# danielbrathwaite/OpenGL-Path-Tracing

Measured on AMD Instinct MI355X. Metric: Mrays/sec + ms/frame @1920×1080, 8 bounces, 1/2/4/8 MI355X, higher is better.
Workload: dtype f32; 1 GPU; C2: cornell 1920x1080, 1024 spp (frames 1..1024), 8 bounces (i<=8), AA+sky+sphere on; scene=cornell, width=1920, height=1080, spp=1024, max_bounce=8, frames_per_launch=1024, kernel_variant=0, parallelism=single GPU

## Files before the change

include/pt_api.h:

```cpp
#ifndef PT_API_H
#define PT_API_H

#include <stddef.h>

#ifdef __cplusplus
extern "C" {
#endif

#define PT_OK 0
#define PT_E_ARG (-1)
#define PT_E_IO (-2)
#define PT_E_PARSE (-3)
#define PT_E_SCENE (-4)
#define PT_E_HIP (-5)
#define PT_E_STATE (-6)

#define PT_FLAG_NO_AA 1
#define PT_FLAG_NO_SKY 2
#define PT_FLAG_NO_SPHERES 4
#define PT_FLAG_NO_TRIANGLES 8
#define PT_FLAG_REF_DISPATCH 16
#define PT_FLAG_MOLLER_TRUMBORE 32
#define PT_FLAG_ALL 63

// ... 26 lines not shown
int pt_progressive_setup(pt_ctx* ctx, int frames_per_launch, int launches_per_replay);
int pt_progressive_reset(pt_ctx* ctx, int next_frame);
int pt_progressive_run(pt_ctx* ctx, int replays);

int pt_rows(const pt_ctx* ctx, int* rows_local, int* row0, int* row_stride);
int pt_get_config(const pt_ctx* ctx, pt_config* out);

int pt_read_rgba32f(pt_ctx* ctx, float* host_dst, size_t bytes);
int pt_read_rgba8_aces(pt_ctx* ctx, unsigned char* host_dst, size_t bytes);
int pt_present_begin(pt_ctx* ctx, int buf);
int pt_present_end(pt_ctx* ctx, int buf, const unsigned char** pixels);
int pt_write_rgba32f(pt_ctx* ctx, const float* host_src, size_t bytes);

int pt_accum_device(pt_ctx* ctx, void** dev_ptr, size_t* bytes);
int pt_copy_rows_device(pt_ctx* ctx, void* dst_dev, size_t bytes);
int pt_stream(pt_ctx* ctx, void** stream);

int pt_set_counting(pt_ctx* ctx, int enable);
int pt_stats(pt_ctx* ctx, double* kernel_ms, unsigned long long out[5]);
int pt_stats_ex(pt_ctx* ctx, unsigned long long out[16]);
int pt_debug_launches(pt_ctx* ctx, unsigned long long out[2]);
int pt_debug_window_cull(pt_ctx* ctx, int* active, float* slack);
int pt_debug_sweep(pt_ctx* ctx, int* swept, int* qualifies, int* n_leaves);
int pt_debug_tile_order(pt_ctx* ctx, unsigned long long* sorts, unsigned* perm_out, int max_tiles, int* n_tiles,
                        int* tiles_x);
int pt_timing(pt_ctx* ctx, double* total_kernel_ms, int* n_launches, int reset);

int pt_set_kernel(pt_ctx* ctx, int variant);
int pt_set_tuning(pt_ctx* ctx, int key, int value);

typedef struct {
    unsigned long long pixels;
    unsigned long long sum_q;
    unsigned long long above;
    unsigned int max_q;
    int frames;
} pt_noise_stats;

int pt_set_moments(pt_ctx* ctx, int enable);
int pt_read_moments(pt_ctx* ctx, float* host_dst, size_t bytes, int* frames);
int pt_noise(pt_ctx* ctx, float target, pt_noise_stats* out);
int pt_noise_host(const float* moments, const unsigned char* in_footprint, size_t n_pixels, int frames,
                  float target, pt_noise_stats* out);
int pt_render_until(pt_ctx* ctx, int frame_first, int accumulate_first, int batch, int max_frames,
                    float target, int* frames_done, pt_noise_stats* last);

// ... 17 lines not shown
```

opengl-path-tracing_amd/csrc/pt_launch_plan.cpp:

```cpp
#include "pt_launch_plan.h"

#include "../../include/pt_api.h"

#include <algorithm>
#include <cmath>

namespace ptl {

static int resident_waves(int minw, bool lds) { return minw ? minw : (lds ? 7 : 6); }

static bool lds_staged(const SceneFacts& f, const Tuning& t, const Image& im, const State& s) {
    if (t.variant == 3) return false;
    if (f.lds_bytes <= kLdsSceneSmall) return true;
    return !s.counting && !t.minw && im.rpp == 1 && f.lds_bytes <= kLdsSceneMax;
}

bool cons_walk_on(const SceneFacts& f, const Tuning& t, bool counting) {
    if (!f.walk_nested || t.cons_off || counting) return false;
    const size_t mw = (size_t)resident_waves(t.minw, true);
    const auto blocks = [mw](size_t b) { return b ? std::min(mw, kLdsCu / b) : mw; };
    return blocks(f.lds_bytes_sk) >= blocks(f.lds_bytes);
}

bool window_cull_on(const SceneFacts& f, const Tuning& t, int flags, bool counting) {
// ... 120 lines not shown
    }
    if (p.overlap && p.nt == 256) {
        const int bpc = t.overlap_bpc ? t.overlap_bpc
                      : t.overlap_slots >= 3 ? (s.aces_fuse ? std::max(1, p.mw - 2) : 3)
                                             : std::max(1, p.mw - 1);
        p.blocks = std::min<unsigned>(p.blocks, (unsigned)(bpc * im.n_cu));
    }
    p.n_top = p.mw > 6 ? std::min(f.n_top, (int)kLdsCu / p.mw / 32 - 8) : f.n_top;
    const size_t shade_bytes = (size_t)(3 * f.n_mats + 2 * f.n_spheres) * 16;
    p.shade_lds = shade_bytes <= 4096;
    const size_t shade_lds_bytes = p.shade_lds ? shade_bytes : 0;
    if (p.wide) {
        const size_t blocks_cu = wide_nt == 1024 ? 1
                               : (wide_nt == 256 ? (size_t)(im.rpp > 1 ? 6 : std::min(std::max(p.mw, 5), 7))
                                                 : (size_t)(6 * 256 / wide_nt));
        p.wide_top = (int)std::min<size_t>({(size_t)f.n_wide, (size_t)kWideTopMax,
                                            (kLdsCu / blocks_cu - shade_lds_bytes - 1024) / 48});
    }
    p.dyn_lds_bytes = p.lds ? lds : (p.wide ? (size_t)p.wide_top * 48 : (size_t)p.n_top * 32) + shade_lds_bytes;
    p.key = kernel_key(s.counting, p.lds, p.wide, p.split, p.mw, im.rpp, p.nt, f.walk_np);
    p.common = !s.adaptive && common_launch(f, t, im, p);
    p.sweep = p.lds && p.nt == 256 && sweep_on(f, t, s.counting);
    if (p.sweep && !t.shade_thresh) p.shade_thresh = kSweepShadeThresh;
    if (p.split) {
        p.accum_long = n_frames > kShortLaunch;
        p.accum_moments = s.moments;
        p.aces_out = s.aces_fuse && !graph;
        const long long px = (long long)im.rows_local * im.width, per_block = 256 * (p.accum_long ? kAccumPixLong : kAccumPix);
        p.accum_blocks = (unsigned)((px + per_block - 1) / per_block);
    }
    return p;
}

size_t scratch_bytes(const LaunchPlan& plan, const Image& im, int n_frames) {
    if (!plan.split) return 0;
    return (size_t)std::max(im.rows_local, 1) * (size_t)im.width * (size_t)n_frames * 3 * sizeof(float);
}

}
```

opengl-path-tracing_amd/csrc/pt_launch_plan.h:

```cpp
#pragma once

#include <stddef.h>

namespace ptl {

#ifndef PT_PAD_NODES
#define PT_PAD_NODES 67
#endif
constexpr int kPadNodes = PT_PAD_NODES;
constexpr unsigned kPullBatch = 32;

constexpr size_t kLdsCu = 160 * 1024;
constexpr size_t kLdsSceneMax = 152 * 1024;
constexpr size_t kLdsSceneSmall = 48 * 1024;
constexpr int kShortLaunch = 16;
constexpr int kWideTopMax = 1 << 14;
constexpr int kWideThreadsAuto = 256;
constexpr int kMaxSlots = 4, kAutoSlots = 3;
#ifndef PT_ACCUM_PIX
#define PT_ACCUM_PIX 4
#endif
constexpr int kAccumPix = PT_ACCUM_PIX, kAccumPixLong = 2;
#ifndef PT_SWEEP_MAX_LEAVES
#define PT_SWEEP_MAX_LEAVES 24
#endif
constexpr int kSweepMaxLeaves = PT_SWEEP_MAX_LEAVES;
static_assert(kSweepMaxLeaves >= 1 && kSweepMaxLeaves <= 32, "a lane's candidate set is one 32-bit mask");
#ifndef PT_SWEEP_SHADE_THRESH
#define PT_SWEEP_SHADE_THRESH 56
#endif
constexpr int kSweepShadeThresh = PT_SWEEP_SHADE_THRESH;

struct SceneFacts {
    int n_nodes = 0, n_spheres = 0, n_mats = 0, n_slots = 0, n_top = 0, walk_np = 1, scene_fast = 0;
    bool walk_nested = false;
    bool wide_ok = false;
    int n_wide = 0;
    bool leaf_cert_ok = false;
    size_t lds_bytes = 0, lds_bytes_sk = 0;
    float root_box[6] = {0, 0, 0, 0, 0, 0};
    int root_child = -1;
    float cons_m[3] = {0, 0, 0};
    float win_slack[3] = {0, 0, 0};
    bool win_bad = false;
    float wide_cw[3] = {0, 0, 0};
    int n_leaves = 0;
    bool sweep_ok = false;
};

struct Tuning {
    int leaf_thresh = 0, shade_thresh = 0, minw = 0, trav_floor = 0, compact_max = 63, pull_batch = 0;
    int group_force = 0;
    int cons_off = 0;
    int wide_off = 0;
    int wide_threads = 0;
    int overlap_bpc = 0;
    int cert_off = 0;
    int overlap_slots = kAutoSlots;
    size_t scratch_budget = 0;
    int variant = 0;
    bool adaptive = true;
    int common_off = 0;
    int win_off = 0;
    int sweep_off = 0;
};

struct Image {
    int width, rows_local, n_tiles, rpp, flags, n_cu;
    unsigned persist_blocks;
    int tile_shift = 0;
};
struct State {
    bool counting, moments, aces_fuse;
    bool adaptive = false;
};

struct KernelKey { bool count, lds; int minw; bool multi, split, padn; int nt; bool wide; };
inline bool operator==(const KernelKey& a, const KernelKey& b) {
    return a.count == b.count && a.lds == b.lds && a.minw == b.minw && a.multi == b.multi && a.split == b.split &&
           a.padn == b.padn && a.nt == b.nt && a.wide == b.wide;
}

struct LaunchPlan {
    bool lds, wide, cons_walk, leaf_cert, split, overlap, shade_lds;
    int nt, mw, group, pull_batch, leaf_thresh, shade_thresh, trav_floor, n_top, wide_top;
    unsigned grp_magic, blocks;
    size_t dyn_lds_bytes;
    bool accum_long, accum_moments, aces_out;
    unsigned accum_blocks;
    KernelKey key;
    bool common;
    bool sweep;
};

constexpr KernelKey kCommonKey = {false, true, 7, false, true, true, 256, false};

bool cons_walk_on(const SceneFacts& f, const Tuning& t, bool counting);
bool window_cull_on(const SceneFacts& f, const Tuning& t, int flags, bool counting);
bool sweep_on(const SceneFacts& f, const Tuning& t, bool counting);
unsigned long long id_limit(const Tuning& t, const Image& im);

LaunchPlan plan_launch(const SceneFacts& f, const Tuning& t, const Image& im, const State& s, int n_frames,
                       bool graph);

int launch_frames(const SceneFacts& f, const Tuning& t, const Image& im, const State& s, int n_frames);

size_t scratch_bytes(const LaunchPlan& plan, const Image& im, int n_frames);

}
```

opengl-path-tracing_amd/csrc/pt_render.hip:

```cpp
#include "pt_cull.h"
#include "pt_isect.h"
#include "pt_launch_plan.h"
#include "pt_math.h"
#include "pt_noise.h"
#include "pt_render_kernels.h"
#include "pt_scene_pack.h"
#include "pt_wide.h"
#include "../../include/pt_api.h"
#include "../../include/pt_scene.h"

#include <hip/hip_runtime.h>

#include <cstdio>
#include <cstring>
#include <string>
#include <vector>

using pt::f3;
using pt::mk;
using ptl::kAccumPix;
using ptl::kAccumPixLong;
using ptl::kPadNodes;
using ptl::kPullBatch;

#include "pt_kparams.h"
#include "pt_render_sm.h"
#include "pt_post_kernels.h"

using ptl::kAutoSlots;
using ptl::kMaxSlots;
using ptl::kShortLaunch;
constexpr int kRingMult = 2, kRingMax = kRingMult * kMaxSlots;
constexpr size_t kQueueSet = kQueueStride;

constexpr int kPresentBufs = 4;

struct pt_ctx {
    pt_config cfg{};
    int rows_local = 0;
    hipStream_t stream = nullptr;
    std::vector<hipEvent_t> ev_free;
    std::vector<std::pair<hipEvent_t, hipEvent_t>> ev_pending;
    double total_ms = 0.0;
    int n_launches = 0;
    float4* accum = nullptr;
    uchar4* rgba8 = nullptr;
    float4* d_scene[ptp::kBufsAll] = {};
    ptl::SceneFacts sf;
    ptl::Tuning tun;
// ... 11 lines not shown
    int order_skip = 0;
    bool order_sorted = false;
    unsigned long long n_sorts = 0, graph_sorts = 0;
    int n_cu = 0;
    float* d_rgb = nullptr;
    size_t rgb_bytes = 0;
    hipStream_t rstream[kMaxSlots] = {};
    float* slot_rgb[kRingMax] = {};
    size_t slot_rgb_bytes[kRingMax] = {};
    hipEvent_t ev_rdone[kRingMax] = {}, ev_adone[kRingMax] = {};
    hipEvent_t ev_fence = nullptr;
    bool adone_rec[kRingMax] = {}, fence_rec = false;
    int slot = 0;
    int ring = 0;
    float* graph_rgb = nullptr;
    std::vector<float*> graph_owned;
    bool scene_ok = false, cam_ok = false, counting = false;
    float cam[12] = {0};
    float last_ms = 0.0f;
    unsigned long long last_counts[16] = {0};
    unsigned long long n_line_launches[2] = {0, 0};
    bool count_pending = false;
    bool last_swept = false;
    unsigned char* present_host[kPresentBufs] = {};
    hipEvent_t ev_copied[kPresentBufs] = {};
    bool present_pending[kPresentBufs] = {};
    bool presented = false, aces_fuse = false, stage_ok = false;
    float2* moments = nullptr;
    int mom_frames = 0;
    pt_noise_stats* d_noise = nullptr;
    pt_noise_stats* h_noise = nullptr;
    bool mom_mixed = false;
    unsigned* d_tile_frames = nullptr;
    unsigned* d_active[2] = {nullptr, nullptr};
    AdaptSum* d_adapt = nullptr;
    AdaptSum* h_adapt = nullptr;
    std::string err;
};

static unsigned pack_tile(const pt_ctx* c, unsigned t) {
    return ((t / (unsigned)c->tiles_x) << 16) | (t % (unsigned)c->tiles_x);
}


static void drop_graph(pt_ctx* c);
static int ensure_tiles(pt_ctx* c);
// ... 212 lines not shown
};
static bool in_0_1(int v) { return v == 0 || v == 1; }
static bool in_0_64(int v) { return v >= 0 && v <= 64; }
static const char kThresholdMsg[] = "threshold must be in 1..64 (0 = automatic)";
static const TuningKey kTuningKeys[] = {
    {0, &ptl::Tuning::leaf_thresh, in_0_64, kThresholdMsg, true},
    {1, &ptl::Tuning::shade_thresh, in_0_64, kThresholdMsg, true},
    {3, nullptr, in_0_64, kThresholdMsg, true},
    {3, &ptl::Tuning::minw, [](int v) { return v == 0 || (v >= 5 && v <= 8); }, "waves per SIMD must be 5..8 (0 = auto)", true},
    {4, &ptl::Tuning::pull_batch, [](int v) { return v >= 0 && v <= 1024; }, "pull batch must be 1..1024 (0 = auto)", true},
    {5, &ptl::Tuning::group_force, [](int v) { return v >= 0; }, "frames per work item must be >= 1 (0 = automatic)", true},
    {6, &ptl::Tuning::trav_floor, in_0_64, kThresholdMsg, true},
    {7, &ptl::Tuning::compact_max, [](int v) { return v >= 0 && v <= 63; }, "compaction limit must be in 0..63", true},
    {15, &ptl::Tuning::cons_off, in_0_1, "culling walk: 0 = automatic, 1 = off", true},
    {16, &ptl::Tuning::wide_off, in_0_1, "wide global walk: 0 = automatic, 1 = off", true},
    {17, &ptl::Tuning::wide_threads, [](int v) { return v == 0 || v == 256 || v == 512 || v == 768 || v == 1024; },
     "wide walk workgroup: 256, 512, 768 or 1024 threads (0 = automatic)", true},
    {18, &ptl::Tuning::overlap_bpc, [](int v) { return v >= 0 && v <= 8; },
     "overlapped render blocks per CU must be 1..8 (0 = automatic)", false},
    {19, &ptl::Tuning::cert_off, in_0_1, "leaf re-test certificate: 0 = automatic, 1 = off", true},
    {21, &ptl::Tuning::common_off, in_0_1, "specialised default-path kernel: 0 = automatic, 1 = off", true},
    {22, &ptl::Tuning::win_off, in_0_1, "window clause of the culling walk: 0 = automatic, 1 = off", true},
    {23, &ptl::Tuning::sweep_off, in_0_1, "leaf sweep: 0 = automatic, 1 = off", true},
};

int pt_set_tuning(pt_ctx* c, int key, int value) {
    if (!c) return PT_E_ARG;
    const TuningKey* hit = nullptr;
    for (const TuningKey& k : kTuningKeys) {
        if (k.key != key) continue;
        if (!k.ok(value)) return fail(c, PT_E_ARG, k.msg);
        hit = &k;
    }
    if (hit) {
        c->tun.*hit->member = value;
        if (hit->drops_graph) drop_graph(c);
        return PT_OK;
    }
    if (key == 8) {
        if (value < 0) return fail(c, PT_E_ARG, "scratch budget (MiB) must be >= 0 (0 = automatic)");
        if (value == 0) {
            size_t total_mem = 0;
            HIPCHK(c, hipDeviceTotalMem(&total_mem, c->cfg.device));
            c->tun.scratch_budget = std::min<size_t>(32ull << 30, total_mem / 4);
        } else {
            c->tun.scratch_budget = (size_t)value << 20;
// ... 186 lines not shown
    const int re = c->ring % ring;
    hipStream_t rs = c->stream;
    unsigned* work = c->d_work;
    if (pl.overlap) {
        int rc = ensure_slot(c, sl, re, scratch);
        if (rc) return rc;
        rs = c->rstream[sl];
        work = c->d_work + kQueueSet * (1 + re);
        p.rgb = c->slot_rgb[re];
        p.work_counter = work;
        c->slot = (sl + 1) % c->tun.overlap_slots;
        c->ring = (re + 1) % ring;
    } else if (pl.split) {
        int rc = ensure_rgb(c, scratch);
        if (rc) return rc;
        p.rgb = c->d_rgb;
    }
    if (c->rows_local == 0) return PT_OK;
    const bool common = pl.common && common_params_ok(c, p, n_frames);
    if (pl.sweep && (!p.sweep_tab || p.n_sweep < 1 || p.n_sweep > ptl::kSweepMaxLeaves || 2 * p.n_sweep != p.n_slots))
        return fail(c, PT_E_STATE, "internal: a sweeping launch without a sweep table");
    const RenderKernel* kernel = find_kernel(pl.key, common, pl.sweep);
    c->last_swept = pl.sweep;
    if (!kernel) {
        const ptl::KernelKey& k = pl.key;
        char key[96];
        std::snprintf(key, sizeof key, "<%d,%d,%d,%d,%d,%d,%d,%d>", k.count, k.lds, k.minw, k.multi, k.split, k.padn, k.nt, k.wide);
        return fail(c, PT_E_STATE, std::string("no k_render_sm instantiation for the launch key ") + key);
    }
    if (pl.overlap) {
        if (c->adone_rec[re]) HIPCHK(c, hipStreamWaitEvent(rs, c->ev_adone[re], 0));
        if (c->fence_rec) HIPCHK(c, hipStreamWaitEvent(rs, c->ev_fence, 0));
    }
    if (pl.overlap) p.reset_work = work;
    else HIPCHK(c, hipMemsetAsync(work, 0, kQueueSet * sizeof(unsigned), rs));
    hipLaunchKernelGGL(kernel->fn, dim3(pl.blocks), dim3((unsigned)kernel->key.nt), pl.dyn_lds_bytes, rs, p);
    c->n_line_launches[common]++;
    if (pl.split) {
        if (pl.overlap) {
            HIPCHK(c, hipEventRecord(c->ev_rdone[re], rs));
            HIPCHK(c, hipStreamWaitEvent(c->stream, c->ev_rdone[re], 0));
        }
        p.aces_out = pl.aces_out ? c->rgba8 : nullptr;
        c->stage_ok = pl.aces_out;
        p.moments = c->moments;
        hipLaunchKernelGGL(accum_kernel(pl), dim3(pl.accum_blocks), dim3(256), 0, c->stream, p);
        if (pl.overlap) {
            HIPCHK(c, hipEventRecord(c->ev_adone[re], c->stream));
            c->adone_rec[re] = true;
        }
    }
    if (p.tile_cost && c->n_tiles > 1 &&
        (frame_dev || force_sort || n_frames > kShortLaunch ||
         ++c->order_skip >= (c->order_sorted ? kOrderEvery : kOrderFirst))) {
        c->order_skip = 0;
        c->order_sorted = true;
        c->n_sorts++;
        hipLaunchKernelGGL(k_tile_order, dim3(1), dim3(1024), 0, c->stream, c->d_tile_cost, c->d_tile_perm,
                           c->n_tiles, c->tiles_x);
// ... 365 lines not shown
}

static int enqueue_adaptive(pt_ctx* c, int frame_first, int n_frames, int acc_first, const unsigned* list, unsigned n_list,
                            unsigned* next, int n_after, unsigned frames_after, unsigned target_q) {
    ptl::Image im = plan_image(c);
    im.n_tiles = (int)n_list;
    ptl::State st = plan_state(c);
    st.adaptive = true;
    const ptl::LaunchPlan pl = ptl::plan_launch(c->sf, c->tun, im, st, n_frames, false);
    if (!pl.split || pl.overlap || pl.common) return fail(c, PT_E_STATE, "internal: an adaptive launch must be a plain split launch");
    KParams p = fill_params(c, pl, frame_first, n_frames, acc_first, nullptr, 0);
    int rc = ensure_rgb(c, ptl::scratch_bytes(pl, plan_image(c), n_frames));
    if (rc) return rc;
    p.rgb = c->d_rgb;
    p.tile_perm = list;
    p.queue_tiles = n_list;
    p.tile_cost = nullptr;
    p.moments = c->moments;
    if (pl.sweep && (!p.sweep_tab || p.n_sweep < 1 || p.n_sweep > ptl::kSweepMaxLeaves || 2 * p.n_sweep != p.n_slots))
        return fail(c, PT_E_STATE, "internal: a sweeping launch without a sweep table");
    const RenderKernel* kernel = find_kernel(pl.key, false, false);
    if (!kernel) return fail(c, PT_E_STATE, "no k_render_sm instantiation for the adaptive launch's key");
    c->last_swept = pl.sweep;
    HIPCHK(c, hipMemsetAsync(c->d_work, 0, kQueueSet * sizeof(unsigned), c->stream));
    hipLaunchKernelGGL(kernel->fn, dim3(pl.blocks), dim3((unsigned)kernel->key.nt), pl.dyn_lds_bytes, c->stream, p);
    c->n_line_launches[0]++;
    const unsigned per_wave = adapt_tiles_per_wave(n_list), per_block = 4u * per_wave;
    AdaptArgs a = {n_list, per_wave, c->n_tiles, n_after, frames_after, target_q, c->d_tile_frames, next, c->d_adapt};
    hipLaunchKernelGGL(k_accum_retire, dim3((n_list + per_block - 1) / per_block), dim3(256), 0, c->stream, p, a);
    HIPCHK(c, hipGetLastError());
    return PT_OK;
}

int pt_render_adaptive(pt_ctx* c, int frame_first, int acc_first, int batch, int max_frames, float target,
                       int* frames_done, pt_adaptive_stats* last) {
    if (!c || !frames_done) return PT_E_ARG;
    *frames_done = 0;
    if (batch < 2 || max_frames < batch || !(target > 0.0f))
        return fail(c, PT_E_ARG, "pt_render_adaptive: batch >= 2, max_frames >= batch, target > 0");
    if (!c->scene_ok) return fail(c, PT_E_STATE, "pt_render_adaptive before pt_upload_scene");
    if (acc_first && c->moments && c->mom_mixed)
        return fail(c, PT_E_STATE, "per-tile frame counts after pt_render_adaptive: the next adaptive call must restart the image");
    if (!c->moments) {
        int rc = pt_set_moments(c, 1);
        if (rc) return rc;
    }
// ... 188 lines not shown
    if (!c || !out) return PT_E_ARG;
    std::memcpy(out, c->last_counts, sizeof(c->last_counts));
    out[13] = c->sf.lds_bytes;
    out[14] = c->sf.walk_nested ? c->sf.lds_bytes_sk : 0;
    out[15] = ptl::cons_walk_on(c->sf, c->tun, c->counting);
    return PT_OK;
}

int pt_debug_window_cull(pt_ctx* c, int* active, float* slack) {
    if (!c) return PT_E_ARG;
    if (active) *active = ptl::window_cull_on(c->sf, c->tun, c->cfg.flags, c->counting) ? 1 : 0;
    if (slack) *slack = std::max(c->sf.win_slack[0], std::max(c->sf.win_slack[1], c->sf.win_slack[2]));
    return PT_OK;
}

int pt_debug_sweep(pt_ctx* c, int* swept, int* qualifies, int* n_leaves) {
    if (!c) return PT_E_ARG;
    if (swept) *swept = c->last_swept ? 1 : 0;
    if (qualifies) *qualifies = c->sf.sweep_ok ? 1 : 0;
    if (n_leaves) *n_leaves = c->sf.n_leaves;
    return PT_OK;
}

int pt_debug_launches(pt_ctx* c, unsigned long long out[2]) {
    if (!c || !out) return PT_E_ARG;
    out[0] = c->n_line_launches[0];
    out[1] = c->n_line_launches[1];
    return PT_OK;
}

int pt_debug_tile_order(pt_ctx* c, unsigned long long* sorts, unsigned* perm_out, int max_tiles, int* n_tiles,
                        int* tiles_x) {
    if (!c) return PT_E_ARG;
    if (perm_out && max_tiles < c->n_tiles) return fail(c, PT_E_ARG, "tile order buffer too small");
    HIPCHK(c, hipSetDevice(c->cfg.device));
    HIPCHK(c, hipStreamSynchronize(c->stream));
    if (sorts) *sorts = c->n_sorts;
    if (n_tiles) *n_tiles = c->n_tiles;
    if (tiles_x) *tiles_x = c->tiles_x;
    if (perm_out && c->n_tiles > 0)
        HIPCHK(c, hipMemcpy(perm_out, c->d_tile_perm, (size_t)c->n_tiles * sizeof(unsigned), hipMemcpyDeviceToHost));
    return PT_OK;
}

int pt_stats(pt_ctx* c, double* ms, unsigned long long out[5]) {
    if (!c) return PT_E_ARG;
// ... 8 lines not shown
```

opengl-path-tracing_amd/pt_host.py:

```python
from __future__ import annotations

import ctypes as C
import os
import subprocess

import numpy as np

PKG_DIR = os.path.dirname(os.path.abspath(__file__))
LIB_PATH = os.environ.get("PT_LIB") or os.path.join(PKG_DIR, "build", "libptrace.so")
INCLUDE_DIR = os.path.join(os.path.dirname(PKG_DIR), "include")

PT_FLAG_NO_AA, PT_FLAG_NO_SKY, PT_FLAG_NO_SPHERES, PT_FLAG_NO_TRIANGLES, PT_FLAG_REF_DISPATCH = 1, 2, 4, 8, 16
PT_FLAG_MOLLER_TRUMBORE = 32
DEFAULT_CAMERA = np.array([0, -6, 1, 0, 0, 1, 0, 0, 0, 0, 0, 0], np.float32)

_ERR = {-1: "PT_E_ARG", -2: "PT_E_IO", -3: "PT_E_PARSE", -4: "PT_E_SCENE", -5: "PT_E_HIP", -6: "PT_E_STATE",
        -7: "PT_E_RCCL"}


class PTError(RuntimeError):
    def __init__(self, code, msg):
        super().__init__("%s (%d): %s" % (_ERR.get(code, "PT_E?"), code, msg))
        self.code = code

# ... 69 lines not shown
            "pt_last_error": (C.c_char_p, [vp]),
            "pt_upload_scene": (ip, [vp, _F, ip, _F, ip, _F, ip, _F, ip]),
            "pt_set_camera": (ip, [vp, _F]),
            "pt_render": (ip, [vp, ip, ip, ip]),
            "pt_render_async": (ip, [vp, ip, ip, ip]),
            "pt_sync": (ip, [vp]),
            "pt_rows": (ip, [vp, C.POINTER(ip), C.POINTER(ip), C.POINTER(ip)]),
            "pt_read_rgba32f": (ip, [vp, vp, C.c_size_t]),
            "pt_read_rgba8_aces": (ip, [vp, vp, C.c_size_t]),
            "pt_write_rgba32f": (ip, [vp, vp, C.c_size_t]),
            "pt_present_begin": (ip, [vp, ip]),
            "pt_present_end": (ip, [vp, ip, C.POINTER(C.POINTER(C.c_ubyte))]),
            "pt_accum_device": (ip, [vp, C.POINTER(vp), C.POINTER(C.c_size_t)]),
            "pt_stream": (ip, [vp, C.POINTER(vp)]),
            "pt_set_counting": (ip, [vp, ip]),
            "pt_stats": (ip, [vp, C.POINTER(C.c_double), np.ctypeslib.ndpointer(np.uint64)]),
            "pt_set_kernel": (ip, [vp, ip]),
            "pt_copy_rows_device": (ip, [vp, vp, C.c_size_t]),
            "pt_timing": (ip, [vp, C.POINTER(C.c_double), C.POINTER(ip), ip]),
            "pt_stats_ex": (ip, [vp, np.ctypeslib.ndpointer(np.uint64)]),
            "pt_debug_launches": (ip, [vp, np.ctypeslib.ndpointer(np.uint64)]),
            "pt_debug_window_cull": (ip, [vp, C.POINTER(ip), C.POINTER(fp)]),
            "pt_debug_sweep": (ip, [vp, C.POINTER(ip), C.POINTER(ip), C.POINTER(ip)]),
            "pt_debug_tile_order": (ip, [vp, C.POINTER(C.c_ulonglong), vp, ip, C.POINTER(ip), C.POINTER(ip)]),
            "pt_set_tuning": (ip, [vp, ip, ip]),
            "pt_progressive_setup": (ip, [vp, ip, ip]),
            "pt_progressive_reset": (ip, [vp, ip]),
            "pt_progressive_run": (ip, [vp, ip]),
            "pt_set_display_mode": (ip, [vp, ip]),
            "pt_get_config": (ip, [vp, C.POINTER(_Config)]),
            "pt_set_moments": (ip, [vp, ip]),
            "pt_read_moments": (ip, [vp, vp, C.c_size_t, C.POINTER(ip)]),
            "pt_noise": (ip, [vp, fp, C.POINTER(NoiseStats)]),
            "pt_noise_host": (ip, [_F, vp, C.c_size_t, ip, fp, C.POINTER(NoiseStats)]),
            "pt_render_until": (ip, [vp, ip, ip, ip, ip, fp, C.POINTER(ip), C.POINTER(NoiseStats)]),
            "pt_group_noise": (ip, [vp, fp, C.POINTER(NoiseStats)]),
            "pt_render_adaptive": (ip, [vp, ip, ip, ip, ip, fp, C.POINTER(ip), C.POINTER(AdaptiveStats)]),
            "pt_read_tile_frames": (ip, [vp, vp, ip, C.POINTER(ip), C.POINTER(ip)]),
            "pt_tile_retires_host": (ip, [_F, vp, C.c_size_t, ip, fp, C.POINTER(ip)]),
            "pt_group_create": (ip, [C.POINTER(vp), ip, C.POINTER(vp)]),
            "pt_group_destroy": (None, [vp]),
            "pt_group_last_error": (C.c_char_p, [vp]),
            "pt_group_upload_scene": (ip, [vp, _F, ip, _F, ip, _F, ip, _F, ip]),
            "pt_group_gather_rgba32f": (ip, [vp, vp, C.c_size_t, ip]),
            "pt_group_stats": (ip, [vp, C.POINTER(C.c_double), C.POINTER(C.c_size_t)]),
            "pt_group_gather_rgba8_aces": (ip, [vp, vp, C.c_size_t, ip]),
# ... 221 lines not shown
        self._check(lib().pt_set_tuning(self.h, 15, 0 if enable else 1))

    def set_common(self, enable):
        self._check(lib().pt_set_tuning(self.h, 21, 0 if enable else 1))

    def set_window_cull(self, enable):
        self._check(lib().pt_set_tuning(self.h, 22, 0 if enable else 1))

    def window_cull(self):
        a, s = C.c_int(), C.c_float()
        self._check(lib().pt_debug_window_cull(self.h, C.byref(a), C.byref(s)))
        return bool(a.value), float(s.value)

    def set_sweep(self, enable):
        self._check(lib().pt_set_tuning(self.h, 23, 0 if enable else 1))

    def leaf_sweep(self):
        a, q, n = C.c_int(), C.c_int(), C.c_int()
        fn = getattr(lib(), "pt_debug_sweep", None)
        if fn is not None:
            self._check(fn(self.h, C.byref(a), C.byref(q), C.byref(n)))
        return dict(swept=bool(a.value), qualifies=bool(q.value), n_leaves=int(n.value))

    def tile_order(self):
        n, tx, sorts = C.c_int(), C.c_int(), C.c_ulonglong()
        self._check(lib().pt_debug_tile_order(self.h, None, None, 0, C.byref(n), None))
        perm = np.zeros(max(n.value, 1), np.uint32)
        self._check(lib().pt_debug_tile_order(self.h, C.byref(sorts), perm.ctypes.data, len(perm), C.byref(n),
                                              C.byref(tx)))
        perm = perm[: n.value]
        return dict(sorts=int(sorts.value), n_tiles=n.value, tiles_x=tx.value,
                    perm=np.stack([perm >> 16, perm & 0xffff], 1).astype(np.int64))

    def launches(self):
        v = np.zeros(2, np.uint64)
        self._check(lib().pt_debug_launches(self.h, v))
        return int(v[0]), int(v[1])

    def set_key(self, key, value):
        self._check(lib().pt_set_tuning(self.h, int(key), int(value)))

    def dispatch(self, frame, accumulate):
        self._check(lib().pt_render(self.h, frame, 1, accumulate))

    def render(self, frame_first, n_frames, accumulate_first):
        self._check(lib().pt_render(self.h, frame_first, n_frames, accumulate_first))
# ... 315 lines not shown
```

Before: 32070 Mrays/s.

## Add wavefront path-pool kernel regrouping shade and leaf-test work per wave

Adds a new render kernel that keeps a per-wave pool of path records in LDS and repeatedly chooses either a shade/trace phase or a leaf-intersection phase, pulling up to 64 paths from two index lists so every lane in a pass does the same kind of work. It is meant to cut SIMD divergence between paths that are shading and paths still testing sweep leaves. It is enabled by default for the common sweep path with one sphere. It costs LDS capacity for path state, LDS round-trips each pass, and a more complex work-queue refill, and it replaces a tuned existing kernel.

```diff
diff --git a/include/pt_api.h b/include/pt_api.h
--- a/include/pt_api.h
+++ b/include/pt_api.h
@@ -72,6 +72,7 @@
 int pt_debug_launches(pt_ctx* ctx, unsigned long long out[2]);
 int pt_debug_window_cull(pt_ctx* ctx, int* active, float* slack);
 int pt_debug_sweep(pt_ctx* ctx, int* swept, int* qualifies, int* n_leaves);
+int pt_debug_pool(pt_ctx* ctx, int* pooled);
 int pt_debug_tile_order(pt_ctx* ctx, unsigned long long* sorts, unsigned* perm_out, int max_tiles, int* n_tiles,
                         int* tiles_x);
 int pt_timing(pt_ctx* ctx, double* total_kernel_ms, int* n_launches, int reset);
diff --git a/opengl-path-tracing_amd/csrc/pt_launch_plan.cpp b/opengl-path-tracing_amd/csrc/pt_launch_plan.cpp
--- a/opengl-path-tracing_amd/csrc/pt_launch_plan.cpp
+++ b/opengl-path-tracing_amd/csrc/pt_launch_plan.cpp
@@ -1,4 +1,6 @@
 #include "pt_launch_plan.h"
+
+#include "pt_pool.h"
 
 #include "../../include/pt_api.h"
 
@@ -166,6 +168,19 @@
     p.common = !s.adaptive && common_launch(f, t, im, p);
     p.sweep = p.lds && p.nt == 256 && sweep_on(f, t, s.counting);
     if (p.sweep && !t.shade_thresh) p.shade_thresh = kSweepShadeThresh;
+    {
+        p.pool_paths = kPoolPaths, p.pool_nt = kPoolThreads;
+        const int wpb = kPoolThreads / 64;
+        const size_t scene = (size_t)(4 * f.n_slots + 3 * f.n_mats + 2 * f.n_spheres + 2 * f.n_leaves) * 16;
+        p.pool_lds_bytes = ptpool::block_bytes(kPoolPaths, wpb, scene);
+        const int full_cu = 4 * kPoolWaves / wpb;
+        const int per_cu = (int)std::min<size_t>(kLdsCu / (p.pool_lds_bytes + 1024), (size_t)full_cu);
+        p.pool = kPoolDefault && !t.pool_off && p.common && p.sweep && !p.overlap && per_cu >= 1 && per_cu == full_cu &&
+                 ptpool::pack_ok(im.width, im.rows_local, n_frames, 0, f.n_slots, f.n_spheres);
+        const unsigned long long paths = (unsigned long long)im.n_tiles * n_groups * 64ull, per_block = (unsigned long long)(kPoolPaths * wpb);
+        p.pool_blocks = (unsigned)std::min<unsigned long long>((unsigned long long)std::max(per_cu, 1) * (unsigned long long)std::max(im.n_cu, 1),
+                                                               std::max(1ull, (paths + per_block - 1) / per_block));
+    }
     if (p.split) {
         p.accum_long = n_frames > kShortLaunch;
         p.accum_moments = s.moments;
diff --git a/opengl-path-tracing_amd/csrc/pt_launch_plan.h b/opengl-path-tracing_amd/csrc/pt_launch_plan.h
--- a/opengl-path-tracing_amd/csrc/pt_launch_plan.h
+++ b/opengl-path-tracing_amd/csrc/pt_launch_plan.h
@@ -30,6 +30,20 @@
 #define PT_SWEEP_SHADE_THRESH 56
 #endif
 constexpr int kSweepShadeThresh = PT_SWEEP_SHADE_THRESH;
+#ifndef PT_POOL_PATHS
+#define PT_POOL_PATHS 116
+#endif
+#ifndef PT_POOL_THREADS
+#define PT_POOL_THREADS 512
+#endif
+#ifndef PT_POOL_WAVES
+#define PT_POOL_WAVES 4
+#endif
+#ifndef PT_POOL_DEFAULT
+#define PT_POOL_DEFAULT 1
+#endif
+constexpr int kPoolPaths = PT_POOL_PATHS, kPoolThreads = PT_POOL_THREADS, kPoolWaves = PT_POOL_WAVES;
+constexpr bool kPoolDefault = PT_POOL_DEFAULT != 0;
 
 struct SceneFacts {
     int n_nodes = 0, n_spheres = 0, n_mats = 0, n_slots = 0, n_top = 0, walk_np = 1, scene_fast = 0;
@@ -63,6 +77,7 @@
     int common_off = 0;
     int win_off = 0;
     int sweep_off = 0;
+    int pool_off = 0;
 };
 
 struct Image {
@@ -91,6 +106,10 @@
     KernelKey key;
     bool common;
     bool sweep;
+    bool pool;
+    int pool_paths, pool_nt;
+    unsigned pool_blocks;
+    size_t pool_lds_bytes;
 };
 
 constexpr KernelKey kCommonKey = {false, true, 7, false, true, true, 256, false};
diff --git a/opengl-path-tracing_amd/csrc/pt_pool.h b/opengl-path-tracing_amd/csrc/pt_pool.h
--- /dev/null
+++ b/opengl-path-tracing_amd/csrc/pt_pool.h
@@ -0,0 +1,65 @@
+#pragma once
+
+#include <stdint.h>
+
+#include "pt_math.h"
+
+namespace ptpool {
+
+constexpr int kLanes = 64;
+constexpr int kMaxPaths = 128;
+constexpr int kRecDwords = 20;
+constexpr int kChunks = kRecDwords / 4;
+
+enum : int { kChunkO = 0, kChunkD = 1, kChunkInc = 2, kChunkCol = 3, kChunkItem = 4 };
+
+PT_HD int quad_of(int c, int i, int P) { return c * P + i; }
+PT_HD int list_bytes(int P) { return (P + 15) & ~15; }
+PT_HD int wave_bytes(int P) { return P * kRecDwords * 4 + list_bytes(P); }
+
+constexpr uint32_t kNoItem = 0xffffffffu;
+PT_HD bool pack_ok(int width, int rows_local, int n_frames, int max_bounce, int n_slots, int n_spheres) {
+    return width >= 1 && width <= 65535 && rows_local >= 0 && rows_local <= 65535 && n_frames >= 1 &&
+           n_frames <= 65535 && max_bounce >= 0 && max_bounce <= 65533 && n_slots >= 0 && n_slots <= 65533 &&
+           n_spheres == 1 && (long long)n_frames * (long long)(max_bounce + 2) < (1ll << 31);
+}
+PT_HD uint32_t pack_xy(int lx, int crow) { return (uint32_t)lx | ((uint32_t)crow << 16); }
+PT_HD int xy_lx(uint32_t v) { return (int)(v & 0xffffu); }
+PT_HD int xy_crow(uint32_t v) { return (int)(v >> 16); }
+PT_HD uint32_t pack_k(int k, int kend) { return (uint32_t)k | ((uint32_t)kend << 16); }
+PT_HD int k_k(uint32_t v) { return (int)(v & 0xffffu); }
+PT_HD int k_kend(uint32_t v) { return (int)(v >> 16); }
+PT_HD uint32_t pack_hit(int hprim, int bounce) { return (uint32_t)(hprim + 2) | ((uint32_t)(bounce + 1) << 16); }
+PT_HD int hit_hprim(uint32_t v) { return (int)(v & 0xffffu) - 2; }
+PT_HD int hit_bounce(uint32_t v) { return (int)(v >> 16) - 1; }
+PT_HD uint32_t with_hprim(uint32_t v, int hprim) { return (v & 0xffff0000u) | (uint32_t)(hprim + 2); }
+PT_HD uint32_t pack_cost(uint32_t pcost, bool report) { return pcost | (report ? 0x80000000u : 0u); }
+PT_HD uint32_t cost_of(uint32_t v) { return v & 0x7fffffffu; }
+PT_HD bool cost_report(uint32_t v) { return (v >> 31) != 0u; }
+
+enum : int { kShade = 0, kLeaf = 1 };
+struct Lists { int nS, nL; };
+
+PT_HD int choose(const Lists& l) { return l.nS >= l.nL ? kShade : kLeaf; }
+PT_HD int take(const Lists& l, int phase) {
+    const int n = phase == kShade ? l.nS : l.nL;
+    return n < kLanes ? n : kLanes;
+}
+PT_HD int pop_index(const Lists& l, int phase, int n, int lane, int P) {
+    return phase == kShade ? l.nS - n + lane : P - l.nL + lane;
+}
+PT_HD void drop(Lists& l, int phase, int n) {
+    if (phase == kShade) l.nS -= n; else l.nL -= n;
+}
+PT_HD int push_index(const Lists& l, int phase, int rank, int P) {
+    return phase == kShade ? l.nS + rank : P - 1 - l.nL - rank;
+}
+PT_HD void grow(Lists& l, int phase, int n) {
+    if (phase == kShade) l.nS += n; else l.nL += n;
+}
+
+PT_HD size_t block_bytes(int P, int waves, size_t scene_bytes) {
+    return ((scene_bytes + 15) & ~(size_t)15) + (size_t)waves * (size_t)wave_bytes(P);
+}
+
+}
diff --git a/opengl-path-tracing_amd/csrc/pt_render.hip b/opengl-path-tracing_amd/csrc/pt_render.hip
--- a/opengl-path-tracing_amd/csrc/pt_render.hip
+++ b/opengl-path-tracing_amd/csrc/pt_render.hip
@@ -3,6 +3,7 @@
 #include "pt_launch_plan.h"
 #include "pt_math.h"
 #include "pt_noise.h"
+#include "pt_pool.h"
 #include "pt_render_kernels.h"
 #include "pt_scene_pack.h"
 #include "pt_wide.h"
@@ -25,6 +26,7 @@
 
 #include "pt_kparams.h"
 #include "pt_render_sm.h"
+#include "pt_render_pool.h"
 #include "pt_post_kernels.h"
 
 using ptl::kAutoSlots;
@@ -82,6 +84,7 @@
     unsigned long long n_line_launches[2] = {0, 0};
     bool count_pending = false;
     bool last_swept = false;
+    bool last_pooled = false;
     unsigned char* present_host[kPresentBufs] = {};
     hipEvent_t ev_copied[kPresentBufs] = {};
     bool present_pending[kPresentBufs] = {};
@@ -340,6 +343,7 @@
     {21, &ptl::Tuning::common_off, in_0_1, "specialised default-path kernel: 0 = automatic, 1 = off", true},
     {22, &ptl::Tuning::win_off, in_0_1, "window clause of the culling walk: 0 = automatic, 1 = off", true},
     {23, &ptl::Tuning::sweep_off, in_0_1, "leaf sweep: 0 = automatic, 1 = off", true},
+    {24, &ptl::Tuning::pool_off, in_0_1, "path pool: 0 = automatic, 1 = off", true},
 };
 
 int pt_set_tuning(pt_ctx* c, int key, int value) {
@@ -572,6 +576,9 @@
         return fail(c, PT_E_STATE, "internal: a sweeping launch without a sweep table");
     const RenderKernel* kernel = find_kernel(pl.key, common, pl.sweep);
     c->last_swept = pl.sweep;
+    const bool pool = pl.pool && common && pl.sweep &&
+                      ptpool::pack_ok(p.W, p.rows_local, n_frames, p.max_bounce, p.n_slots, p.sc.n_spheres);
+    c->last_pooled = pool;
     if (!kernel) {
         const ptl::KernelKey& k = pl.key;
         char key[96];
@@ -584,7 +591,11 @@
     }
     if (pl.overlap) p.reset_work = work;
     else HIPCHK(c, hipMemsetAsync(work, 0, kQueueSet * sizeof(unsigned), rs));
-    hipLaunchKernelGGL(kernel->fn, dim3(pl.blocks), dim3((unsigned)kernel->key.nt), pl.dyn_lds_bytes, rs, p);
+    if (pool)
+        hipLaunchKernelGGL((k_render_pool<ptl::kPoolThreads, ptl::kPoolPaths, ptl::kPoolWaves>), dim3(pl.pool_blocks),
+                           dim3((unsigned)pl.pool_nt), pl.pool_lds_bytes, rs, p);
+    else
+        hipLaunchKernelGGL(kernel->fn, dim3(pl.blocks), dim3((unsigned)kernel->key.nt), pl.dyn_lds_bytes, rs, p);
     c->n_line_launches[common]++;
     if (pl.split) {
         if (pl.overlap) {
@@ -996,6 +1007,7 @@
     const RenderKernel* kernel = find_kernel(pl.key, false, false);
     if (!kernel) return fail(c, PT_E_STATE, "no k_render_sm instantiation for the adaptive launch's key");
     c->last_swept = pl.sweep;
+    c->last_pooled = false;
     HIPCHK(c, hipMemsetAsync(c->d_work, 0, kQueueSet * sizeof(unsigned), c->stream));
     hipLaunchKernelGGL(kernel->fn, dim3(pl.blocks), dim3((unsigned)kernel->key.nt), pl.dyn_lds_bytes, c->stream, p);
     c->n_line_launches[0]++;
@@ -1230,6 +1242,12 @@
     return PT_OK;
 }
 
+int pt_debug_pool(pt_ctx* c, int* pooled) {
+    if (!c) return PT_E_ARG;
+    if (pooled) *pooled = c->last_pooled ? 1 : 0;
+    return PT_OK;
+}
+
 int pt_debug_launches(pt_ctx* c, unsigned long long out[2]) {
     if (!c || !out) return PT_E_ARG;
     out[0] = c->n_line_launches[0];
diff --git a/opengl-path-tracing_amd/csrc/pt_render_pool.h b/opengl-path-tracing_amd/csrc/pt_render_pool.h
--- /dev/null
+++ b/opengl-path-tracing_amd/csrc/pt_render_pool.h
@@ -0,0 +1,318 @@
+namespace {
+
+__device__ __forceinline__ void pool_cold_walk(const KParams& p, const SceneView& S, f3 o, f3 d, float& t, int& hprim) {
+    int w = 0;
+    while (w >= 0) {
+        const float4 lo = p.sc.nodes[2 * w], hi = p.sc.nodes[2 * w + 1];
+        const int a = __float_as_int(hi.z), b = __float_as_int(hi.w);
+        if (!slab(lo, hi, o, d, t)) { w = b; continue; }
+        if (a >= 0) { w = a; continue; }
+        const int q = (~a) >> 2;
+        const int s0 = 2 * __float_as_int(p.sweep_tab[2 * q + 1].w);
+        const bool cop = __float_as_int(tri_quad<true>(S, s0 + 1, 1).w) != 0;
+        const float4 nda = tri_quad<true>(S, s0, 0);
+        const float4 ndb = cop ? nda : tri_quad<true>(S, s0 + 1, 0);
+        const float ta = tri_plane(nda, o, d);
+        const float tb = cop ? ta : tri_plane(ndb, o, d);
+        bool oka = false, okb = false, ca = false, cb = false;
+        if (win_open(ta, t)) oka = tri_edges_at<true, false>(S, s0, mk(nda.x, nda.y, nda.z), o + d * ta, false, 0.0f, ca);
+        if (win_closed(tb, t)) okb = tri_edges_at<true, false>(S, s0 + 1, mk(ndb.x, ndb.y, ndb.z), o + d * tb, false, 0.0f, cb);
+        const float h1 = oka ? ta : -1.0f, h2 = okb ? tb : -1.0f;
+        const bool c1 = win_open(h1, t) & ((h1 < h2) | (h2 < 0.0001f));
+        const bool c2 = !c1 & win_open(h2, t);
+        if (c1 | c2) {
+            t = c1 ? h1 : h2;
+            hprim = s0 + (c1 ? 0 : 1);
+        }
+        w = b;
+    }
+}
+
+__device__ __forceinline__ void pool_pass_fence() {
+    __builtin_amdgcn_fence(__ATOMIC_RELEASE, "wavefront");
+    __builtin_amdgcn_wave_barrier();
+    __builtin_amdgcn_fence(__ATOMIC_ACQUIRE, "wavefront");
+}
+
+template <int NT, int P, int MINW>
+__global__ __launch_bounds__(NT, MINW) void k_render_pool(KParams p) {
+    static_assert(P >= 64 && P <= ptpool::kMaxPaths && P % 4 == 0, "one-byte list entries in a 16-byte padded array");
+    using namespace ptpool;
+    const const_v4f* const sweep_tab = (const const_v4f*)(size_t)p.sweep_tab;
+    resolve_frames(p);
+    extern __shared__ float4 lds[];
+    const int T = p.n_slots, nt = 4 * T, nm = 3 * p.n_mats, ns = 2, nb = 2 * p.n_sweep;
+    for (int i = threadIdx.x; i < nt; i += NT) {
+        const int slot = i >> 2, c = __float_as_int(p.sweep_tab[2 * (slot >> 1) + 1].w);
+        lds[(i & 3) * T + 2 * c + (slot & 1)] = p.sc.tris[i];
+    }
+    for (int i = threadIdx.x; i < nm; i += NT) lds[nt + i] = p.sc.mats[i];
+    for (int i = threadIdx.x; i < ns; i += NT) lds[nt + nm + i] = p.sc.spheres[i];
+    for (int i = threadIdx.x; i < nb; i += NT) lds[nt + nm + ns + i] = p.sweep_tab[i];
+    const int scene_q = nt + nm + ns + nb;
+    const int lane = (int)(threadIdx.x & 63u);
+    float4* const pool = lds + scene_q + (int)(threadIdx.x >> 6) * (wave_bytes(P) / 16);
+    unsigned char* const list = (unsigned char*)(pool + kChunks * P);
+    for (int i = lane; i < P; i += kLanes) {
+        pool[quad_of(kChunkO, i, P)] = make_float4(0, 0, 0, -1.0f);
+        pool[quad_of(kChunkD, i, P)] = make_float4(0, 0, 1, 0);
+        pool[quad_of(kChunkInc, i, P)] = make_float4(0, 0, 0, __uint_as_float(pack_hit(-1, -1)));
+        pool[quad_of(kChunkCol, i, P)] = make_float4(1, 1, 1, 0);
+        pool[quad_of(kChunkItem, i, P)] = make_float4(__uint_as_float(kNoItem), 0, 0, 0);
+        list[i] = (unsigned char)i;
+    }
+    __syncthreads();
+    SceneView S;
+    S.nodes = nullptr;
+    S.tris = lds;
+    S.mats = lds + nt;
+    S.spheres = lds + nt + nm;
+    const float4* const boxes = lds + nt + nm + ns;
+    S.np = 0;
+    S.tp = T;
+    S.cm[0] = p.cons_m[0], S.cm[1] = p.cons_m[1], S.cm[2] = p.cons_m[2];
+    S.ws[0] = p.win_slack[0], S.ws[1] = p.win_slack[1], S.ws[2] = p.win_slack[2];
+    S.clo = ptc::kWindowLo;
+    const f3 cpos = mk(p.cam[0], p.cam[1], p.cam[2]), cfwd = mk(p.cam[3], p.cam[4], p.cam[5]);
+    const f3 cright = mk(p.cam[6], p.cam[7], p.cam[8]), cup = mk(p.cam[9], p.cam[10], p.cam[11]);
+    const int tiles_x = (p.W + 7) >> 3;
+    const unsigned n_groups = (unsigned)((p.n_frames + p.group - 1) / p.group);
+    const unsigned total_ids = p.queue_tiles * n_groups * 64u;
+    unsigned qnext = 0, qend = 0;
+    Lists L = {P, 0};
+    while (L.nS + L.nL > 0) {
+        const int phase = choose(L), n = take(L, phase);
+        const bool on = lane < n;
+        int idx = 0;
+        if (on) idx = list[pop_index(L, phase, n, lane, P)];
+        drop(L, phase, n);
+        bool to_shade = false, to_leaf = false;
+        if (phase == kShade) {
+            const float4 c0 = pool[quad_of(kChunkO, idx, P)], c1 = pool[quad_of(kChunkD, idx, P)];
+            const float4 c2 = pool[quad_of(kChunkInc, idx, P)], c3 = pool[quad_of(kChunkCol, idx, P)];
+            const float4 c4 = pool[quad_of(kChunkItem, idx, P)];
+            f3 o = mk(c0.x, c0.y, c0.z), d = mk(c1.x, c1.y, c1.z), inc = mk(c2.x, c2.y, c2.z), col = mk(c3.x, c3.y, c3.z);
+            float t = c0.w;
+            unsigned bi = __float_as_uint(c1.w);
+            int hprim = hit_hprim(__float_as_uint(c2.w)), bounce = hit_bounce(__float_as_uint(c2.w));
+            uint32_t state = __float_as_uint(c3.w);
+            unsigned xy = __float_as_uint(c4.x);
+            int aidx = __float_as_int(c4.y);
+            int k = k_k(__float_as_uint(c4.z)), kend = k_kend(__float_as_uint(c4.z));
+            unsigned pcost = cost_of(__float_as_uint(c4.w));
+            bool report = cost_report(__float_as_uint(c4.w));
+            bool retired = false;
+            if (on && !(t < 0.0f)) {
+                const bool hit = hprim != -1;
+                pcost++;
+                bool finished = false;
+                f3 rgb = inc;
+                if (hit && pt::length_gt_001(col)) {
+                    const f3 hitp = o + d * t;
+                    f3 normal;
+                    int mat;
+                    if (hprim >= 0) {
+                        const float4 nq = tri_quad<true>(S, hprim, 0);
+                        normal = mk(nq.x, nq.y, nq.z);
+                        mat = __float_as_int(tri_quad<true>(S, hprim, 2).w);
+                    } else {
+                        const int si = -2 - hprim;
+                        float4 s0 = S.spheres[2 * si];
+                        normal = pt::normalize(hitp - mk(s0.x, s0.y, s0.z));
+                        mat = __float_as_int(S.spheres[2 * si + 1].x);
+                    }
+                    if (pt::dot(normal, d) > 0.0f) normal = normal * -1.0f;
+                    o = hitp;
+                    f3 diffuse = pt::normalize(normal + pt::random_unit_vector(state));
+                    float kk = 2.0f * pt::dot(normal, d);
+                    f3 specular = pt::normalize(d - normal * kk);
+                    float4 m0 = S.mats[3 * mat], m1 = S.mats[3 * mat + 1], m2 = S.mats[3 * mat + 2];
+                    float is_spec = (m1.w > pt::random01(state)) ? 1.0f : 0.0f;
+                    d = pt::mix(diffuse, specular, m0.w * is_spec);
+                    inc = inc + mk(m1.x, m1.y, m1.z) * col;
+                    col = col * pt::mix(mk(m0.x, m0.y, m0.z), mk(m2.x, m2.y, m2.z), is_spec);
+                    bounce++;
+                    if (bounce > p.max_bounce) {
+                        rgb = inc;
+                        finished = true;
+                    }
+                } else {
+                    f3 dir = pt::normalize(d);
+                    float tt = 0.5f * (dir.z + 1.0f);
+                    float omt = 1.0f - tt;
+                    f3 env = mk(omt * 1.0f + tt * 0.5f, omt * 1.0f + tt * 0.7f, omt * 1.0f + tt * 1.0f);
+                    rgb = inc + env * col;
+                    finished = true;
+                }
+                if (finished) {
+                    bounce = -1;
+                    const f3 px = (mk(0, 0, 0) + rgb) / 1.0f;
+                    nt_store3(p.rgb + 3 * ((size_t)k * (size_t)(p.rows_local * p.W) + (size_t)aidx), px);
+                    k++;
+                }
+                t = -1.0f;
+            }
+            if (on & (bounce < 0) & (xy != kNoItem) & (k >= kend)) {
+                if (report) atomicAdd(&p.tile_cost[(xy_crow(xy) >> 3) * tiles_x + (xy_lx(xy) >> 3)], pcost);
+                xy = kNoItem;
+            }
+            const bool want = on && xy == kNoItem;
+            const unsigned long long m = __ballot(want);
+            if (m) {
+                const unsigned need = (unsigned)__popcll(m);
+                const unsigned rank = (unsigned)rank_in(m);
+                const int leader = __ffsll((long long)m) - 1;
+                unsigned id;
+                if (qend - qnext >= need) {
+                    id = qnext + rank;
+                    qnext += need;
+                } else {
+                    const unsigned avail = qend - qnext;
+                    const unsigned take_ids = max(need - avail, (unsigned)p.pull_batch);
+                    unsigned base = 0;
+                    if (want && rank == 0u) base = atomicAdd(p.work_counter, take_ids);
+                    base = (unsigned)__builtin_amdgcn_readlane((int)base, leader);
+                    id = rank < avail ? qnext + rank : base + (rank - avail);
+                    qnext = base + (need - avail);
+                    qend = base + take_ids;
+                }
+                if (want) {
+                    if (id >= total_ids) {
+                        retired = true;
+                    } else {
+                        const unsigned item = id >> 6, w = id & 63u;
+                        const unsigned tile = p.grp_magic ? __umulhi(item, p.grp_magic) : item;
+                        const int g = (int)(item - tile * n_groups);
+                        const unsigned pk = p.tile_perm[tile];
+                        const int tx = (int)(pk & 0xffffu), ty = (int)(pk >> 16);
+                        const int cx = tx * 8 + (int)(w & 7u);
+                        const int crow = ty * 8 + (int)(w >> 3);
+                        if ((cx < p.W) & (crow < p.rows_local)) {
+                            xy = pack_xy(cx, crow);
+                            aidx = crow * p.W + cx;
+                            report = (w & 0x1bu) == 0u;
+                            pcost = 0;
+                            k = g * p.group;
+                            kend = min(k + p.group, p.n_frames);
+                            bounce = -1;
+                        }
+                    }
+                }
+            }
+            if (on && xy != kNoItem) {
+                const int lx = xy_lx(xy), y = p.row0 + xy_crow(xy) * p.row_stride;
+                if (bounce < 0) {
+                    state = pt::seed(lx, y, p.frame_first + k);
+                    const float ax = pt::random01(state);
+                    const float ay = pt::random01(state);
+                    float u = pt::div_mk((float)lx + ax, p.fW, p.rW) - 0.5f;
+                    float v = pt::div_mk((float)y + ay, p.fH, p.rH) - 0.5f;
+                    d = pt::normalize((cfwd + cright * u) + cup * v);
+                    o = cpos;
+                    inc = mk(0, 0, 0);
+                    col = mk(1, 1, 1);
+                    bounce = 0;
+                }
+                const bool fast_seg =
+                       in_guard(o.x, 0x1p-40f, 0x1p60f) & in_guard(o.y, 0x1p-40f, 0x1p60f) &
+                       in_guard(o.z, 0x1p-40f, 0x1p60f) & in_range_abs(d.x, 0x1p-20f, 2.0f) &
+                       in_range_abs(d.y, 0x1p-20f, 2.0f) & in_range_abs(d.z, 0x1p-20f, 2.0f);
+                const f3 rd = fast_seg ? mk(pt::rcp_fast(d.x), pt::rcp_fast(d.y), pt::rcp_fast(d.z)) : mk(0, 0, 0);
+                t = __builtin_huge_valf();
+                hprim = -1;
+                {
+                    float4 s0 = S.spheres[0];
+                    f3 oc = o - mk(s0.x, s0.y, s0.z);
+                    float a = pt::dot(d, d);
+                    float half_b = pt::dot(oc, d);
+                    float cq = pt::dot(oc, oc) - s0.w;
+                    float disc = half_b * half_b - a * cq;
+                    float ht = disc < 0.0f ? -1.0f : (-half_b - pt::sqrt_g(disc)) / a;
+                    if (win_open(ht, t)) {
+                        t = ht;
+                        hprim = -2;
+                    }
+                }
+                const bool walk = !ray_has_nan(o, d);
+                unsigned cand = 0u;
+                if (walk & fast_seg) {
+                    f3 ol, oh;
+                    ptc::cull_addends(o, rd, S.cm, S.ws, ol, oh);
+                    const ptc::SweepRay sr = ptc::sweep_ray(rd, ol, oh);
+                    bool in = true;
+                    if (p.sweep_root) in = ptc::sweep_root_hit(p.root_box, sr, t, S.clo);
+                    if (in) cand = ptc::sweep_mask(sr, t, S.clo, sweep_tab, p.n_sweep);
+                }
+                const bool cold = walk & !fast_seg;
+                if (__any(cold)) {
+                    if (cold) pool_cold_walk(p, S, o, d, t, hprim);
+                }
+                bi = cand;
+                to_leaf = cand != 0u;
+            }
+            to_shade = on & !retired & !to_leaf;
+            if (on) {
+                pool[quad_of(kChunkO, idx, P)] = make_float4(o.x, o.y, o.z, t);
+                pool[quad_of(kChunkD, idx, P)] = make_float4(d.x, d.y, d.z, __uint_as_float(bi));
+                pool[quad_of(kChunkInc, idx, P)] = make_float4(inc.x, inc.y, inc.z, __uint_as_float(pack_hit(hprim, bounce)));
+                pool[quad_of(kChunkCol, idx, P)] = make_float4(col.x, col.y, col.z, __uint_as_float(state));
+                pool[quad_of(kChunkItem, idx, P)] = make_float4(__uint_as_float(xy), __int_as_float(aidx),
+                                                                __uint_as_float(pack_k(k, kend)),
+                                                                __uint_as_float(pack_cost(pcost, report)));
+            }
+        } else {
+            const float4 c0 = pool[quad_of(kChunkO, idx, P)], c1 = pool[quad_of(kChunkD, idx, P)];
+            float* const hw = (float*)&pool[quad_of(kChunkInc, idx, P)] + 3;
+            const unsigned hb = __float_as_uint(*hw);
+            const f3 o = mk(c0.x, c0.y, c0.z), d = mk(c1.x, c1.y, c1.z);
+            float t = c0.w;
+            unsigned bi = __float_as_uint(c1.w);
+            const bool at = on;
+            int s0 = 0, lp = 0;
+            bool cop = false;
+            float4 nd0 = make_float4(0, 0, 0, 0);
+            if (at) {
+                lp = __ffs((int)bi) - 1;
+                s0 = 2 * lp;
+                cop = __float_as_int(tri_quad<true>(S, s0 + 1, 1).w) != 0;
+                nd0 = tri_quad<true>(S, s0, 0);
+            }
+            float h1 = -1.0f, h2 = -1.0f;
+            bool ca = false, cb = false;
+            leaf_pair_tests<true, false>(S, at, s0, nd0, cop, o, d, t, p.compact_max, h1, h2, false, ca, cb);
+            bool c1h = false, c2h = false;
+            if (at) {
+                c1h = win_open(h1, t) & ((h1 < h2) | (h2 < 0.0001f));
+                c2h = !c1h & win_open(h2, t);
+            }
+            const bool chk = at & (c1h | c2h);
+            if (__any(chk)) {
+                if (chk) {
+                    const f3 rd = mk(pt::rcp_fast(d.x), pt::rcp_fast(d.y), pt::rcp_fast(d.z));
+                    if (!slab_fast(boxes[2 * lp], boxes[2 * lp + 1], o, d, rd, t)) c1h = c2h = false;
+                }
+            }
+            if (at) {
+                int hprim = hit_hprim(hb);
+                if (c1h | c2h) {
+                    t = c1h ? h1 : h2;
+                    hprim = s0 + (c1h ? 0 : 1);
+                }
+                bi &= bi - 1u;
+                to_leaf = bi != 0u;
+                to_shade = bi == 0u;
+                ((float*)&pool[quad_of(kChunkO, idx, P)])[3] = t;
+                ((float*)&pool[quad_of(kChunkD, idx, P)])[3] = __uint_as_float(bi);
+                *hw = __uint_as_float(with_hprim(hb, hprim));
+            }
+        }
+        const unsigned long long mS = __ballot(to_shade), mL = __ballot(to_leaf);
+        if (to_shade) list[push_index(L, kShade, rank_in(mS), P)] = (unsigned char)idx;
+        if (to_leaf) list[push_index(L, kLeaf, rank_in(mL), P)] = (unsigned char)idx;
+        grow(L, kShade, __popcll(mS));
+        grow(L, kLeaf, __popcll(mL));
+        pool_pass_fence();
+    }
+}
+
+}
diff --git a/opengl-path-tracing_amd/pt_host.py b/opengl-path-tracing_amd/pt_host.py
--- a/opengl-path-tracing_amd/pt_host.py
+++ b/opengl-path-tracing_amd/pt_host.py
@@ -115,6 +115,7 @@
             "pt_debug_launches": (ip, [vp, np.ctypeslib.ndpointer(np.uint64)]),
             "pt_debug_window_cull": (ip, [vp, C.POINTER(ip), C.POINTER(fp)]),
             "pt_debug_sweep": (ip, [vp, C.POINTER(ip), C.POINTER(ip), C.POINTER(ip)]),
+            "pt_debug_pool": (ip, [vp, C.POINTER(ip)]),
             "pt_debug_tile_order": (ip, [vp, C.POINTER(C.c_ulonglong), vp, ip, C.POINTER(ip), C.POINTER(ip)]),
             "pt_set_tuning": (ip, [vp, ip, ip]),
             "pt_progressive_setup": (ip, [vp, ip, ip]),
@@ -382,6 +383,16 @@
             self._check(fn(self.h, C.byref(a), C.byref(q), C.byref(n)))
         return dict(swept=bool(a.value), qualifies=bool(q.value), n_leaves=int(n.value))
 
+    def set_pool(self, enable):
+        self._check(lib().pt_set_tuning(self.h, 24, 0 if enable else 1))
+
+    def pooled(self):
+        a = C.c_int()
+        fn = getattr(lib(), "pt_debug_pool", None)
+        if fn is not None:
+            self._check(fn(self.h, C.byref(a)))
+        return bool(a.value)
+
     def tile_order(self):
         n, tx, sorts = C.c_int(), C.c_int(), C.c_ulonglong()
         self._check(lib().pt_debug_tile_order(self.h, None, None, 0, C.byref(n), None))
```

After: 35050 Mrays/s, median of 6. 1.09x the previous value.
